# snarkify/sirius

Measured on AMD Instinct MI355X. Metric: IVC fold-steps/s (CycleFold IVC::next hot path, Poseidon-shaped synthetic trace, 2^k rows), higher is better.
Workload: dtype u256 (modular; 9 x 29-bit / 8 x 32-bit limbs)

## Files before the change

### sirius_amd/csrc/capi.hip

```cpp
#include "../../include/sirius_amd.h"

#include <cstdio>
#include <cstring>
#include <deque>
#include <map>
#include <memory>
#include <set>
#include <thread>
#include <condition_variable>
#include <functional>
#include <mutex>
#include <atomic>
#include <chrono>
#include <string>
#include <vector>

#include "curve.cuh"
#include "decider.h"
#include "devrt.h"
#include "msm.h"
#include "ntt.h"
#include "poseidon.h"
#include "prof.h"
#include "rowprog.h"
// ... 1659 lines not shown
    std::vector<std::pair<size_t, size_t>> runs;
    const std::vector<size_t> need = shard_halo_rows(S, reference_compat);
    for (size_t i = 0; i < need.size();) {
        size_t j = i + 1;
        while (j < need.size() && need[j] == need[j - 1] + 1) ++j;
        runs.emplace_back(need[i], need[j - 1] + 1);
        i = j;
    }
    return guarded([&]() -> int {
        const fe_t *src = reinterpret_cast<const fe_t *>(witness_host);
        fe_t *dst = reinterpret_cast<fe_t *>(dev_copy);
        for (auto &r : runs)
            SRS_HIP_CHECK(hipMemcpy2DAsync(dst + r.first, rows * sizeof(fe_t), src + r.first, rows * sizeof(fe_t), (r.second - r.first) * sizeof(fe_t),
                                           cols, hipMemcpyHostToDevice, (hipStream_t)stream));
        return SRS_OK;
    });
}
size_t srs_structure_num_cross_terms(const srs_structure *S) { return S ? rowprog::degree(S->s) : 0; }
size_t srs_structure_num_challenges(const srs_structure *S) { return S ? rowprog::num_challenges(S->s) : 0; }
size_t srs_structure_num_witness_columns(const srs_structure *S) { return S ? rowprog::num_witness_columns(S->s) : 0; }
int srs_jit_selfcheck(size_t *code_bytes, char *log, size_t log_cap) {
    if constexpr (rt::kEmulated) return fail(SRS_ERR_INVALID, "srs_jit_selfcheck: not part of the emulator build");
    std::string text;
    const bool ok = rowprog::jit_selfcheck(code_bytes, text);
    if (log && log_cap) {
        const size_t n = std::min(text.size(), log_cap - 1);
        std::memcpy(log, text.data(), n);
        log[n] = 0;
    }
    return ok ? SRS_OK : fail(SRS_ERR_INVALID, "srs_jit_selfcheck: hiprtc rejected the emitted form: " + text.substr(0, 400));
}

int srs_structure_kernel_kind(const srs_structure *S, int which) {
    if (!S || which < 0 || which > 2) return -1;
    return rowprog::kernel_kind(S->s, which);
}

size_t srs_structure_program_source(srs_structure *S, int which, char *buf, size_t cap, uint64_t *fingerprint, int *spec_id) {
    if (!S) return 0;
    std::string src;
    rowprog::spec_source(S->s, which, fingerprint, spec_id, src);
    if (buf && cap) {
        size_t n = std::min(src.size(), cap - 1);
        std::memcpy(buf, src.data(), n);
        buf[n] = 0;
    }
    return src.size();
}

static int cross_terms_impl(srs_structure *S, srs_ck *ck, const srs_fe *W1, const srs_fe *W2, const srs_fe *challenges,
                            size_t n_challenges, int space, void *stream, srs_fe *const *T_out, srs_affine *commits_out) {
    if (!S || !W1 || !W2 || (n_challenges && !challenges)) return fail(SRS_ERR_INVALID, "srs_cross_terms: bad argument");
    if (ck && !commits_out) return fail(SRS_ERR_INVALID, "srs_commit_cross_terms: commits_out is NULL");
    int rc = ensure_device();
    if (rc) return rc;
    return guarded([&]() -> int {
        hipStream_t st = (hipStream_t)stream;
        rowprog::Structure *s = S->s;
        const size_t d = rowprog::degree(s), rows = rowprog::rows(s), wlen = rowprog::num_witness_columns(s) * rows;
        if (d == 0) return SRS_OK;
        if (ck && rows > ck->key.global_len)
            return fail(SRS_ERR_TOO_LONG_INPUT, "Can't commit too long input: input len: " + std::to_string(rows) +
                                                    ", but limit is " + std::to_string(ck->key.global_len));
        const bool host = space != SRS_SPACE_DEVICE;
        const bool own_T = host || !T_out;
        size_t need = 1024;
        if (host) need += 2 * Arena::pad(wlen * sizeof(fe_t));
// ... 588 lines not shown
                 srs_fe *W_folded) {
    if (!S || !betas || !delta || !W || !alpha_gamma || !poly_F || !poly_K || !betas_stroke || !e || !lagrange ||
        (n_challenges && !challenges))
        return fail(SRS_ERR_INVALID, "srs_pg_prove: bad argument");
    if (n_instances < 2) return fail(SRS_ERR_INVALID, "You can't fold 0 traces");
    if (n_instances & (n_instances - 1)) return fail(SRS_ERR_INVALID, "instances_to_fold must be a power of two");
    if (ro && ro->h->field != SRS_FIELD_FR) return fail(SRS_ERR_INVALID, "srs_pg_prove: the oracle must be over bn256::Fr");
    if (rowprog::shard_world(S->s) > 1)
        return fail(SRS_ERR_INVALID, "srs_pg_prove: structure is row-sharded (srs_structure_set_shard); use the step-wise calls and add the ranks' polynomials");
    int rc = ensure_device();
    if (rc) return rc;
    return guarded([&]() -> int {
        HostTrace ht("srs_pg_prove");
        hipStream_t st = (hipStream_t)stream;
        rowprog::Structure *s = S->s;
        rowprog::PgSizes z;
        if (!rowprog::pg_sizes(s, n_instances - 1, z)) return fail(SRS_ERR_INVALID, "structure has no gates");
        if (n_betas < z.betas_count) return fail(SRS_ERR_INVALID, "srs_pg_prove: not enough betas");
        if (z.log_domain_K > ntt::FR_S)
            return fail(SRS_ERR_K_TOO_LARGE, "srs_pg_prove (compute_K_from_G): k=" + std::to_string(z.log_domain_K) + " should no larger than F::S=28");
        const size_t wlen = rowprog::num_witness_columns(s) * rowprog::rows(s);
        std::vector<const fe_t *> dW(n_instances), ch(n_instances);
        for (size_t j = 0; j < n_instances; ++j) {
            dW[j] = reinterpret_cast<const fe_t *>(W[j]);
            ch[j] = n_challenges ? reinterpret_cast<const fe_t *>(challenges[j]) : nullptr;
        }
        std::string err;
        size_t n_out = 0;
        const bool closed = rowprog::pg_closed_route(reference_compat);
        const uint32_t n_gates = (uint32_t)rowprog::num_gates(s), levels = (uint32_t)z.betas_count, log_rows = rowprog::log_rows(s);
        rowprog::PgRow0 r0;
        int erc = 0;
        if (closed) {
            erc = rowprog::pg_row0_values(s, true, dW.data(), ch.data(), n_challenges, n_instances, st, r0, err);
            if (erc) return fail(erc, "srs_pg_prove (gates at row 0): " + err);
            ht.mark("row0");
            std::vector<fe_t> c0(n_gates);
            for (uint32_t g = 0; g < n_gates; ++g) c0[g] = r0.vals[(size_t)g * r0.P + r0.one_at];
            rowprog::pg_closed_F(c0.data(), n_gates, log_rows, reinterpret_cast<const fe_t *>(betas), *reinterpret_cast<const fe_t *>(delta), levels,
                                 reinterpret_cast<fe_t *>(poly_F), z.points_F);
        } else {
            erc = rowprog::pg_sum(s, 0, dW.data(), ch.data(), n_challenges, 1, reinterpret_cast<const fe_t *>(betas), n_betas,
                                  reinterpret_cast<const fe_t *>(delta), reference_compat, st, reinterpret_cast<fe_t *>(poly_F), &n_out, err);
            if (erc) return fail(erc, "srs_pg_prove (compute_F): " + err);
        }
        ht.mark("compute_F");
        fe_t alpha, gamma;
        std::memcpy(&alpha, &alpha_gamma[0], 32);
        std::memcpy(&gamma, &alpha_gamma[1], 32);
        if (ro) {
            poseidon::absorb(*ro->h, reinterpret_cast<const fe_t *>(poly_F), z.points_F);
            if (!poseidon::squeeze(*ro->h, 255, SRS_FIELD_FR, alpha, err)) return fail(SRS_ERR_INVALID, "srs_pg_prove (alpha): " + err);
        }
        std::vector<fe_t> bs(z.betas_count);
        {
            fe_t d;
            std::memcpy(&d, delta, 32);
            for (size_t i = 0; i < z.betas_count; ++i) {
                fe_t b;
                std::memcpy(&b, &betas[i], 32);
                bs[i] = Fr::add(b, Fr::mul(alpha, d));
                d = Fr::sqr(d);
            }
        }
        const fe_t f_alpha = rowprog::poly_eval(reinterpret_cast<const fe_t *>(poly_F), z.points_F, alpha);
        ht.mark("alpha,betas'");
        std::vector<fe_t> poly_G(z.points_G);
        rowprog::PgGValues gv;
        const bool k_on_device = n_instances == 2 && z.log_domain_K <= 12;
        std::vector<fe_t> g_vals;
        if (closed)
            rowprog::pg_closed_G(s, r0, bs.data(), levels, poly_G.data(), poly_G.size(), &g_vals);
        else
            erc = rowprog::pg_sum(s, 1, dW.data(), ch.data(), n_challenges, n_instances, bs.data(), bs.size(), nullptr, reference_compat, st,
                                  poly_G.data(), &n_out, err, &f_alpha, k_on_device ? &gv : nullptr);
        if (erc) return fail(erc, "srs_pg_prove (compute_G): " + err);
        if (gv.vals_dev && !rowprog::pg_K_device_ok(gv, z.log_domain_K)) return fail(SRS_ERR_DEVICE, "srs_pg_prove: internal (device K on an unsupported shape)");
        ht.mark("compute_G");
        if (closed && k_on_device && r0.g_int && g_vals.size() <= 32)
            erc = rowprog::pg_K_from_G_values(s, g_vals.data(), (uint32_t)g_vals.size(), f_alpha, z.instances_to_fold, z.log_domain_K, st,
                                              reinterpret_cast<fe_t *>(poly_K), err);
        else if (gv.vals_dev)
            erc = rowprog::pg_K_from_G_device(s, gv, f_alpha, z.instances_to_fold, z.log_domain_K, st, reinterpret_cast<fe_t *>(poly_K), err);
        else
            erc = rowprog::pg_K_from_G(poly_G.data(), poly_G.size(), f_alpha, z.instances_to_fold, z.log_domain_K, st,
                                       reinterpret_cast<fe_t *>(poly_K), err);
        if (erc) return fail(erc, "srs_pg_prove (compute_K_from_G): " + err);
        ht.mark("compute_K");
        const size_t n_K = (size_t)1 << z.log_domain_K;
        if (ro) {
            poseidon::absorb(*ro->h, reinterpret_cast<const fe_t *>(poly_K), n_K);
            if (!poseidon::squeeze(*ro->h, 255, SRS_FIELD_FR, gamma, err)) return fail(SRS_ERR_INVALID, "srs_pg_prove (gamma): " + err);
        }
        ht.mark("gamma");
        const std::vector<fe_t> L = rowprog::lagrange_eval(gamma, (uint32_t)z.lagrange_domain);
        const fe_t zg = Fr::sub(Fr::pow_u64(gamma, (uint64_t)1 << z.lagrange_domain), Fr::one());
        const fe_t kg = rowprog::poly_eval(reinterpret_cast<const fe_t *>(poly_K), n_K, gamma);
        const fe_t ev = Fr::add(Fr::mul(f_alpha, L[0]), Fr::mul(zg, kg));
        if (W_folded) {
            erc = rowprog::lincomb(SRS_FIELD_FR, reinterpret_cast<fe_t *>(W_folded), dW.data(), L.data(), n_instances, wlen, st, err);
            if (erc) return fail(erc, "srs_pg_prove (fold_witness): " + err);
        }
        std::memcpy(&alpha_gamma[0], &alpha, 32);
        std::memcpy(&alpha_gamma[1], &gamma, 32);
        std::memcpy(betas_stroke, bs.data(), bs.size() * sizeof(fe_t));
        std::memcpy(e, &ev, 32);
        std::memcpy(lagrange, L.data(), n_instances * sizeof(fe_t));
        ht.mark("e,L,fold");
        return SRS_OK;
    });
}

static int sangria_prove_impl(srs_structure *S, srs_ck *ck, srs_poseidon *ro, const srs_fe *challenges, size_t n_challenges, srs_fe *W1, srs_fe *W2,
                              const srs_fe *W2_host, const srs_fe *u2_tail, size_t n_u2_tail, srs_fe *E, void *stream, srs_fe *r_io,
                              srs_fe *const *T_dev, srs_affine *cross_term_commits, srs_affine *W_commitments, const srs_affine *E_commitment,
                              srs_affine *folded_commitments, uint64_t *jobs, bool incoming) {
    if (!S || !ck || !W1 || !W2 || !E || !r_io || !T_dev || !cross_term_commits || !W_commitments || !E_commitment || !folded_commitments || !jobs ||
        (n_u2_tail && !u2_tail))
        return fail(SRS_ERR_INVALID, "srs_sangria_prove: bad argument");
    const int curve = ck->key.curve, sf = srs_scalar_field_of(curve);
    if (ro && ro->h->field != (curve == SRS_CURVE_BN256 ? SRS_FIELD_FQ : SRS_FIELD_FR))
// ... 146 lines not shown
```

### sirius_amd/csrc/rowprog.h

```cpp
#pragma once
#include <memory>
#include <string>
#include <vector>

#include "devrt.h"
#include "field.cuh"
#include "rowprog_dev.cuh"

namespace srs {
namespace rowprog {

struct Structure;

Structure *create(int field, uint32_t k, size_t num_selectors, size_t num_fixed, size_t num_advice,
                  const uint8_t *const *selectors, const fe_t *const *fixed, int space_device,
                  const uint64_t *gates, size_t gates_words, size_t num_gates, size_t num_lookups, bool has_vector_lookup,
                  const uint64_t *lookup_exprs, size_t lookup_words, int &rc, std::string &err);
void destroy(Structure *S);
void set_shard(Structure *S, uint32_t rank, uint32_t world);
uint32_t shard_world(const Structure *S);
uint32_t shard_rank(const Structure *S);
void rotation_range(const Structure *S, int32_t *lo, int32_t *hi);
uint32_t log_rows(const Structure *S);
size_t degree(const Structure *S);
size_t num_challenges(const Structure *S);
size_t num_advice(const Structure *S);
size_t num_witness_columns(const Structure *S);
size_t num_lookups(const Structure *S);
size_t rows(const Structure *S);
int field(const Structure *S);

int evaluate(Structure *S, int mode, const fe_t *W1_dev, const fe_t *W2_dev, const fe_t *challenges_host, size_t n_ch,
             fe_t *const *out_dev_ptrs_host, hipStream_t st, std::string &err, bool sync = true);

struct PgSizes {
    size_t count_with_padding = 0, betas_count = 0, points_F = 0, points_G = 0, instances_to_fold = 0, lagrange_domain = 0;
    uint32_t log_domain_K = 0;
};
bool pg_sizes(const Structure *S, size_t traces_len, PgSizes &out);
std::vector<fe_t> lagrange_eval(const fe_t &X, uint32_t log_n);
fe_t poly_eval(const fe_t *coeffs, size_t n, const fe_t &x);
struct PgRow0 {
    std::vector<fe_t> vals;
    uint32_t P = 0, one_at = 0;
    bool g_int = false;
};
bool pg_closed_route(int compat);
int pg_row0_values(Structure *S, bool fold, const fe_t *const *W_dev, const fe_t *const *challenges_host, size_t n_ch, size_t J, hipStream_t st,
                   PgRow0 &out, std::string &err);
fe_t pg_closed_sum(const fe_t *c, size_t stride, uint32_t n_gates, uint32_t k, const fe_t *w, uint32_t levels);
void pg_closed_F(const fe_t *c, uint32_t n_gates, uint32_t k, const fe_t *betas, const fe_t &delta, uint32_t levels, fe_t *out, size_t n_out);
void pg_closed_G(const Structure *S, const PgRow0 &r0, const fe_t *betas_stroke, uint32_t levels, fe_t *out, size_t n_out,
                 std::vector<fe_t> *point_values = nullptr);
size_t num_gates(const Structure *S);
struct PgGValues {
    const fe_t *vals_dev = nullptr;
    uint32_t n_dev = 0, degree = 0;
    bool skip_one = false;
};
int pg_sum(Structure *S, int mode, const fe_t *const *W_dev, const fe_t *const *challenges_host, size_t n_ch, size_t J,
           const fe_t *weights_in, size_t n_weights, const fe_t *delta, int compat, hipStream_t st, fe_t *out_host,
           size_t *n_out, std::string &err, const fe_t *g_at_one = nullptr, PgGValues *keep_on_device = nullptr);
bool pg_K_device_ok(const PgGValues &g, uint32_t log_domain_K);
int pg_K_from_G_device(Structure *S, const PgGValues &g, const fe_t &f_alpha, size_t instances_to_fold, uint32_t log_domain_K, hipStream_t st,
                       fe_t *out_host, std::string &err);
int pg_K_from_G_values(Structure *S, const fe_t *vals_host, uint32_t n, const fe_t &f_alpha, size_t instances_to_fold, uint32_t log_domain_K,
                       hipStream_t st, fe_t *out_host, std::string &err);
int pg_K_from_G(const fe_t *polyG_host, size_t nG, const fe_t &f_alpha, size_t instances_to_fold, uint32_t log_domain_K,
                hipStream_t st, fe_t *out_host, std::string &err);
int lincomb(int field, fe_t *out, const fe_t *const *w_dev, const fe_t *coefs, size_t J, size_t n, hipStream_t st, std::string &err,
            uint32_t rank = 0, uint32_t world = 1);
int lincomb_rows(int field, fe_t *out, const fe_t *const *w_dev, const fe_t *coefs, size_t J, const uint32_t *rows_dev, size_t n_rows, size_t cols,
                 size_t col_len, hipStream_t st, std::string &err);

const char *spec_source(Structure *S, int which, uint64_t *fingerprint, int *spec_id, std::string &buf);
int kernel_kind(const Structure *S, int which);
bool jit_selfcheck(size_t *code_bytes, std::string &log);

int lookup_coeff_1(Structure *S, const fe_t *advice_dev, const fe_t &r, fe_t *const *ls, fe_t *const *ts, fe_t *const *ms,
                   hipStream_t st, std::string &err);
void lookup_coeff_2(int field, const fe_t *l, const fe_t *t, const fe_t *m, const fe_t &r, size_t n, fe_t *h, fe_t *g, hipStream_t st);
size_t log_derivative_mismatches(Structure *S, const fe_t *W_dev, hipStream_t st);
void assigned_invert(int field, const fe_t *num, const fe_t *den, const uint8_t *has_den, size_t n, fe_t *out, hipStream_t st);

size_t count_mismatch(const fe_t *a_dev, const fe_t *b_dev , size_t n, hipStream_t st);

void fold_w(int field, fe_t *out, const fe_t *w1, const fe_t *w2, const fe_t &r, size_t n, hipStream_t st);
int fold_e(int field, fe_t *out, const fe_t *e, const fe_t *const *t_dev_ptrs_host, size_t n_terms, const fe_t &r, size_t n,
           hipStream_t st, std::string &err);

}
}
```

### sirius_amd/csrc/rowprog.hip

```cpp
#include "rowprog.h"
#include "rowprog_compile.h"
#include "ntt.h"
#include "prof.h"
#include "jit.h"
#include "tuning.h"

#include <algorithm>
#include <cstring>
#include <map>
#include <mutex>
#include <tuple>

namespace srs {
namespace rowprog {

template <class F>
__device__ __forceinline__ fe_t interp(fe_t *slots, const Insn *__restrict__ prog, uint32_t n_insn, uint32_t result,
                                       const RowCtx &C, uint32_t row, uint32_t pt, const fe_t *__restrict__ U) {
    const uint32_t tid = threadIdx.x, nthr = blockDim.x, mask = C.rows - 1;
    for (uint32_t ip = 0; ip < n_insn; ++ip) {
        const Insn in = prog[ip];
        fe_t r;
        if (in.op <= I_LD_ADV) {
            uint32_t rr = (row + (uint32_t)(int32_t)in.b) & mask;
            if (in.op == I_LD_SEL) r = ld_sel<F>(C, in.a, rr);
            else if (in.op == I_LD_FIX) r = ld_fix<F>(C, in.a, rr);
            else r = ld_adv<F>(C, in.a, rr, pt);
        } else {
            fe_t a = (in.a & UNIFORM_BIT) ? U[in.a & ~UNIFORM_BIT] : slots[in.a * nthr + tid];
            if (in.op <= I_MUL) {
                fe_t b = (in.b & UNIFORM_BIT) ? U[in.b & ~UNIFORM_BIT] : slots[in.b * nthr + tid];
                r = in.op == I_ADD ? F::add(a, b) : (in.op == I_SUB ? F::sub(a, b) : F::mul(a, b));
            } else if (in.op == I_SQR) {
                r = F::sqr(a);
// ... 668 lines not shown
        "    const fe_t l0 = ld_fix<F>(C, 0, (row + 0u) & mask);\n"
        "    fe_t l1, s1; adv_affine<F>(C, 0, (row + 1u) & mask, l1, s1);\n"
        "    for (uint32_t pt = 0; pt < npts; ++pt) {\n"
        "        const fe_t *__restrict__ U = Uall + (size_t)pt * nu;\n"
        "        const f29_t x0 = G::unpack(l0), x1 = G::unpack(l1);\n"
        "        const f29_t x2 = mul29_ni<F>(x0, x1);\n"
        "        const f29_t x3 = sqr29_ni<F>(x2);\n"
        "        const f29_t x4 = G::normalize(G::template sub_lazy<3, 0>(G::normalize(G::add_lazy(x3, x2)), x3));\n"
        "        const f29_t x5 = G::mul(x4, G::unpack(U[0]));\n"
        "        sw_store(acc, pt, accumulate ? G::normalize(G::add_lazy(sw_load(acc, pt), x5)) : x5);\n"
        "        l1 = F::add(l1, s1);\n    }\n}\n";
    for (int field = 0; field < 2; ++field) {
        size_t bytes = 0;
        if (!jit::compile_only(jit_translation_unit(fn, field, true), &bytes, log)) return false;
        if (code_bytes) *code_bytes = bytes;
    }
    return true;
}

struct Structure : Compiled {
    int field = 0;
    uint32_t k = 0;
    size_t rows = 0, num_selectors = 0, num_fixed = 0, num_advice = 0;
    size_t num_lookups = 0;
    bool has_vector_lookup = false;
    int pg_spec_id = -1;
    GateProg *d_gate_progs = nullptr;
    uint8_t **d_sel_ptrs = nullptr;
    fe_t **d_fix_ptrs = nullptr;
    std::vector<void *> owned;
    fe_t *d_vinv = nullptr, *d_vinv29 = nullptr;
    fe_t *d_kM[2] = {nullptr, nullptr};
    Arena arena;
    std::vector<uint8_t> host_stage;
    uint32_t shard_rank = 0, shard_world = 1;
};

static int match_spec(const Program &p) {
    if (!p.sweep_ok) return -1;
    int id = -1;
    for (size_t i = 0; i < sizeof(kSpecs) / sizeof(kSpecs[0]); ++i)
        if (kSpecs[i].fingerprint == p.fingerprint && kSpecs[i].id >= 0) id = kSpecs[i].id;
    return id;
}

static void *resident(Structure &S, const void *src, size_t bytes, hipMemcpyKind kind = hipMemcpyHostToDevice, size_t spare = 0) {
    void *d = nullptr;
    SRS_HIP_CHECK(hipMalloc(&d, bytes + spare));
    S.owned.push_back(d);
    if (bytes) SRS_HIP_CHECK(hipMemcpy(d, src, bytes, kind));
    return d;
}

Structure *create(int field, uint32_t k, size_t num_selectors, size_t num_fixed, size_t num_advice,
                  const uint8_t *const *selectors, const fe_t *const *fixed, int space_device,
                  const uint64_t *gates, size_t gates_words, size_t num_gates, size_t num_lookups, bool has_vector_lookup,
                  const uint64_t *lookup_exprs, size_t lookup_words, int &rc, std::string &err) {
    std::unique_ptr<Structure, void (*)(Structure *)> S(new Structure(), &destroy);
    if (!compile_structure(field, num_selectors, num_fixed, num_advice, gates, gates_words, num_gates, num_lookups, has_vector_lookup,
                           lookup_exprs, lookup_words, *S, rc, err))
        return nullptr;
    S->field = field;
    S->k = k;
    S->rows = (size_t)1 << k;
    S->num_selectors = num_selectors;
    S->num_fixed = num_fixed;
// ... 22 lines not shown
    }
    rc = 5;
    auto upload_program = [&](Program &p) {
        if (!p.insns.empty()) p.d_insns = (Insn *)resident(*S, p.insns.data(), p.insns.size() * sizeof(Insn));
    };
    for (auto &lp : S->lookup_progs) upload_program(lp);
    upload_program(S->cross);
    upload_program(S->plain_compressed);
    upload_program(S->plain_homogeneous);
    for (auto &gp : S->gate_progs) upload_program(gp);
    if (!S->vinv.empty()) {
        S->d_vinv = (fe_t *)resident(*S, S->vinv.data(), S->vinv.size() * sizeof(fe_t));
        const FieldOps f{field};
        std::vector<fe_t> v29(S->vinv);
        for (auto &x : v29)
            for (int k = 0; k < 5; ++k) x = f.add(x, x);
        S->d_vinv29 = (fe_t *)resident(*S, v29.data(), v29.size() * sizeof(fe_t));
    }
    const hipMemcpyKind kind = space_device ? hipMemcpyDeviceToDevice : hipMemcpyHostToDevice;
    std::vector<uint8_t *> selp(num_selectors);
    std::vector<fe_t *> fixp(num_fixed);
    for (size_t i = 0; i < num_selectors; ++i) selp[i] = (uint8_t *)resident(*S, selectors[i], S->rows, kind);
    for (size_t i = 0; i < num_fixed; ++i) fixp[i] = (fe_t *)resident(*S, fixed[i], S->rows * sizeof(fe_t), kind);
    S->d_sel_ptrs = (uint8_t **)resident(*S, selp.data(), num_selectors * sizeof(void *), hipMemcpyHostToDevice, sizeof(void *));
    S->d_fix_ptrs = (fe_t **)resident(*S, fixp.data(), num_fixed * sizeof(void *), hipMemcpyHostToDevice, sizeof(void *));
    rc = 0;
    return S.release();
}

void destroy(Structure *S) {
    if (!S) return;
    jit::release(S->cross.jit);
    for (void *p : S->owned) (void)hipFree(p);
    S->arena.release();
    delete S;
}

void set_shard(Structure *S, uint32_t rank, uint32_t world) {
    S->shard_rank = rank;
    S->shard_world = world ? world : 1;
}
uint32_t shard_world(const Structure *S) { return S->shard_world; }
uint32_t shard_rank(const Structure *S) { return S->shard_rank; }
void rotation_range(const Structure *S, int32_t *lo, int32_t *hi) { *lo = S->min_rot; *hi = S->max_rot; }
uint32_t log_rows(const Structure *S) { return S->k; }
size_t degree(const Structure *S) { return S->degree; }
size_t num_challenges(const Structure *S) { return S->s_num_challenges; }
size_t num_advice(const Structure *S) { return S->num_advice; }
size_t num_witness_columns(const Structure *S) { return S->num_advice + 5 * S->num_lookups; }
size_t num_lookups(const Structure *S) { return S->num_lookups; }
size_t rows(const Structure *S) { return S->rows; }
size_t num_gates(const Structure *S) { return S->gate_progs.size(); }
int field(const Structure *S) { return S->field; }

template <class F>
static void launch_rowprog(const DevArgs &A, uint32_t nslots, hipStream_t st) {
    uint32_t blocks = (A.ctx.local_rows + RP_THREADS - 1) / RP_THREADS;
    if (nslots <= 8) SRS_LAUNCH((k_rowprog<F, 8>), (blocks), (RP_THREADS), 0, st, A);
    else if (nslots <= 10) SRS_LAUNCH((k_rowprog<F, 10>), (blocks), (RP_THREADS), 0, st, A);
    else if (nslots <= 12) SRS_LAUNCH((k_rowprog<F, 12>), (blocks), (RP_THREADS), 0, st, A);
    else if (nslots <= 16) SRS_LAUNCH((k_rowprog<F, 16>), (blocks), (RP_THREADS), 0, st, A);
    else if (nslots <= 24) SRS_LAUNCH((k_rowprog<F, 24>), (blocks), (RP_THREADS), 0, st, A);
    else SRS_LAUNCH((k_rowprog<F, 32>), (blocks), (RP_THREADS), 0, st, A);
}

int kernel_kind(const Structure *S, int which) {
    if (which == 2) return S->pg_spec_id >= 0 ? 1 : 0;
    const Program &p = which == 0 ? S->cross : S->plain_compressed;
    if (p.spec_id >= 0) return 1;
    if (p.jit.function) return 2;
    return 0;
}

const char *spec_source(Structure *S, int which, uint64_t *fingerprint, int *spec_id, std::string &buf) {
    if (which >= 3 && (size_t)(which - 3) >= S->gate_progs.size()) { buf.clear(); return buf.c_str(); }
    Program &p = which >= 3 ? S->gate_progs[which - 3] : (which == 0 ? S->cross : (which == 1 ? S->plain_compressed : S->plain_homogeneous));
    buf = emit_spec_source(p, "spec_fn", false);
    buf += emit_sweep_source(p, "spec_fn_sweep", false);
    if (fingerprint) *fingerprint = p.fingerprint;
    if (spec_id) *spec_id = p.spec_id;
    if (spec_id && p.spec_id < 0 && p.jit.function) *spec_id = -2;
    return buf.c_str();
}

static int evaluate_prog(Structure *S, Program &p, int mode, const fe_t *W1_dev, const fe_t *W2_dev, const fe_t *challenges_host,
                         size_t n_ch, fe_t *const *out_dev_ptrs_host, hipStream_t st, std::string &err, bool sync = true);
int evaluate(Structure *S, int mode, const fe_t *W1_dev, const fe_t *W2_dev, const fe_t *challenges_host, size_t n_ch,
             fe_t *const *out_dev_ptrs_host, hipStream_t st, std::string &err, bool sync) {
    Program &p = mode == 0 ? S->cross : (mode == 1 ? S->plain_compressed : S->plain_homogeneous);
    return evaluate_prog(S, p, mode, W1_dev, W2_dev, challenges_host, n_ch, out_dev_ptrs_host, st, err, sync);
}
static int evaluate_prog(Structure *S, Program &p, int mode, const fe_t *W1_dev, const fe_t *W2_dev, const fe_t *challenges_host,
                         size_t n_ch, fe_t *const *out_dev_ptrs_host, hipStream_t st, std::string &err, bool sync) {
    FieldOps f{S->field};
    const uint32_t d = mode == 0 ? (uint32_t)S->degree : 0;
    const uint32_t npts = mode == 0 ? d + 1 : 1;
    const uint32_t nout = mode == 0 ? d : 1;
    if (mode == 0 && d == 0) return 0;
    if (p.nslots > 32) { err = "row program needs more than 32 live registers"; return 4; }
// ... 182 lines not shown
    uint32_t deg = levels > k ? levels - k : 0;
    for (uint32_t b = 0; b < k && b < levels; ++b) mul_linear(sum, deg, Fr::add(Fr::one(), betas[b]), deltas[b]);
    for (size_t m = 0; m < n_out; ++m) out[m] = m <= deg ? sum[m] : Fr::zero();
}

void pg_closed_G(const Structure *S, const PgRow0 &r0, const fe_t *betas_stroke, uint32_t levels, fe_t *out, size_t n_out, std::vector<fe_t> *point_values) {
    const uint32_t n_gates = (uint32_t)S->gate_progs.size(), P = r0.P;
    std::vector<fe_t> val(P);
    for (uint32_t p = 0; p < P; ++p) val[p] = pg_closed_sum(r0.vals.data() + p, P, n_gates, S->k, betas_stroke, levels);
    if (point_values) *point_values = val;
    for (size_t m = 0; m < n_out; ++m) out[m] = Fr::zero();
    if (r0.g_int) {
        const uint32_t dG = P - 1;
        FieldOps f{0};
        const std::vector<fe_t> vinv = !S->vinv_g.empty() ? S->vinv_g : (dG ? inverse_vandermonde_rows(f, dG) : std::vector<fe_t>());
        out[0] = val[0];
        for (uint32_t k = 1; k <= dG && k < n_out; ++k) {
            fe_t acc = Fr::zero();
            for (uint32_t j = 0; j < P; ++j) acc = Fr::add(acc, Fr::mul(vinv[(size_t)(k - 1) * P + j], val[j]));
            out[k] = acc;
        }
        return;
    }
    const fe_t winv = ntt::omega(ilog2(P), true), inv_P = Fr::inv(Fr::from_u64(P));
    fe_t wk = Fr::one();
    for (uint32_t k = 0; k < P && k < n_out; ++k) {
        fe_t acc = Fr::zero(), x = Fr::one();
        for (uint32_t p = 0; p < P; ++p) { acc = Fr::add(acc, Fr::mul(val[p], x)); x = Fr::mul(x, wk); }
        out[k] = Fr::mul(acc, inv_P);
        wk = Fr::mul(wk, winv);
    }
}

int pg_row0_values(Structure *S, bool fold, const fe_t *const *W_dev, const fe_t *const *challenges_host, size_t n_ch, size_t J, hipStream_t st,
                   PgRow0 &out, std::string &err) {
    if (S->field != 0) { err = "ProtoGalaxy polynomials need the 2-adic field bn256::Fr"; return 4; }
    if (J == 0 || J > JMAX) { err = "unsupported number of traces"; return 4; }
    PgSizes sz;
    if (!pg_sizes(S, fold ? J - 1 : 1, sz)) { err = "structure has no gates"; return 4; }
    FieldOps f{0};
    const bool g_int = fold && J == 2 && tuning::get_or(tuning::PG_G_FFT, 0) == 0;
    const uint32_t P = !fold ? 1u : (g_int ? (uint32_t)S->max_gate_degree + 1 : (uint32_t)sz.points_G);
    const uint32_t n_gates = (uint32_t)S->gate_progs.size();
    out.P = P;
    out.g_int = g_int;
    out.one_at = g_int ? 1u : 0u;
    std::vector<fe_t> wcoef;
    std::vector<std::vector<fe_t>> ch_pt(P, std::vector<fe_t>(n_ch ? n_ch : 1, Fr::zero()));
    if (fold) {
        wcoef.resize((size_t)P * J);
        const fe_t w = g_int ? Fr::one() : ntt::omega(ilog2(P), false);
        fe_t x = g_int ? Fr::zero() : Fr::one();
        for (uint32_t p = 0; p < P; ++p) {
            if (!g_int || n_ch) {
                std::vector<fe_t> L = lagrange_eval(x, (uint32_t)sz.lagrange_domain);
                for (size_t j = 0; j < J; ++j) {
                    wcoef[(size_t)p * J + j] = L[j];
                    for (size_t c = 0; c < n_ch; ++c)
                        ch_pt[p][c] = Fr::add(ch_pt[p][c], Fr::mul(challenges_host[j][c], L[j]));
                }
            }
            x = g_int ? Fr::add(x, Fr::one()) : Fr::mul(x, w);
        }
    } else {
        for (size_t c = 0; c < n_ch; ++c) ch_pt[0][c] = challenges_host[0][c];
    }
    const bool sweep = S->pg_spec_id >= 0 && S->k >= 10 && (!fold || g_int) && P <= DMAX + 1;
    const uint32_t lpt = 8;
    uint32_t max_slots = 1;
    std::vector<GateProg> gp(n_gates);
    std::vector<fe_t> utab;
    for (uint32_t g = 0; g < n_gates; ++g) {
        Program &p = S->gate_progs[g];
        max_slots = std::max(max_slots, p.nslots);
        const size_t nu = p.uops.size() ? p.uops.size() : 1;
        gp[g].prog = p.d_insns;
        gp[g].n_insn = (uint32_t)p.insns.size();
        gp[g].result = p.result;
        gp[g].n_uniform = (uint32_t)nu;
        gp[g].utab_off = (uint32_t)utab.size();
        utab.resize(utab.size() + nu * P * (sweep ? lpt + 1 : 1u));
        fe_t *tab = utab.data() + gp[g].utab_off;
        for (uint32_t lp = 0; lp < P; ++lp)
            if (!eval_uniform(p, f, ch_pt[lp].data(), n_ch, 0, false, 0, tab + (size_t)lp * nu, err)) return 7;
        if (sweep) std::memcpy(tab + (size_t)lpt * P * nu, tab, (size_t)P * nu * sizeof(fe_t));
    }
    if (max_slots > 32) { err = "row program needs more than 32 live registers"; return 4; }
    Arena &A = S->arena;
    A.reserve(Arena::pad((wcoef.size() + 1) * sizeof(fe_t)) + Arena::pad((utab.size() + 1) * sizeof(fe_t)) + Arena::pad(gp.size() * sizeof(GateProg)) +
              Arena::pad(((size_t)n_gates * P + 1) * sizeof(fe_t)) + 4096);
    A.reset();
    fe_t *d_coef = A.take<fe_t>(wcoef.size() + 1);
    fe_t *d_utab = A.take<fe_t>(utab.size() + 1);
    GateProg *d_gp = A.take<GateProg>(gp.size());
    fe_t *d_vals = A.take<fe_t>((size_t)n_gates * P + 1);
    if (fold && !g_int) SRS_HIP_CHECK(hipMemcpyAsync(d_coef, wcoef.data(), wcoef.size() * sizeof(fe_t), hipMemcpyHostToDevice, st));
    SRS_HIP_CHECK(hipMemcpyAsync(d_utab, utab.data(), utab.size() * sizeof(fe_t), hipMemcpyHostToDevice, st));
    SRS_HIP_CHECK(hipMemcpyAsync(d_gp, gp.data(), gp.size() * sizeof(GateProg), hipMemcpyHostToDevice, st));
    PgArgs a;
// ... 532 lines not shown
    bool zero_z = false;
    const fe_t *tab = k_domain_table_dev(log_domain_K, instances_to_fold, zero_z);
    if (zero_z) { err = "Z(X) must be not equal to 0"; return 4; }
    fe_t *&M = S->d_kM[g.skip_one ? 1 : 0];
    if (!M) {
        FieldOps f{0};
        std::vector<fe_t> full((size_t)n_nodes * n_nodes);
        if (g.skip_one) {
            full = !S->vinv_g1.empty() ? S->vinv_g1 : inverse_vandermonde_at(f, g.degree, 1);
        } else {
            const std::vector<fe_t> rows = !S->vinv_g.empty() ? S->vinv_g : (g.degree ? inverse_vandermonde_rows(f, g.degree) : std::vector<fe_t>());
            for (uint32_t j = 0; j < n_nodes; ++j) full[j] = j == 0 ? Fr::one() : Fr::zero();
            for (size_t i = 0; i < rows.size(); ++i) full[n_nodes + i] = rows[i];
        }
        SRS_HIP_CHECK(hipMalloc((void **)&M, full.size() * sizeof(fe_t)));
        S->owned.push_back(M);
        SRS_HIP_CHECK(hipMemcpy(M, full.data(), full.size() * sizeof(fe_t), hipMemcpyHostToDevice));
    }
    static thread_local ThreadArena scratch;
    scratch.reserve(Arena::pad((size_t)count * sizeof(fe_t)) + 256);
    scratch.reset();
    fe_t *d_out = scratch.take<fe_t>(count);
    const uint32_t threads = std::max<uint32_t>(64u, std::min<uint32_t>(256u, count));
    SRS_LAUNCH(k_pg_K_small, ((count + threads - 1) / threads), (threads), 0, st, g.vals_dev, g.n_dev, f_alpha, g.skip_one ? 1 : 0, (const fe_t *)M,
               n_nodes, f_alpha, tab, count, d_out);
    ntt::run(d_out, log_domain_K, count, 1, true, true, st);
    SRS_HIP_CHECK(hipMemcpyAsync(out_host, d_out, (size_t)count * sizeof(fe_t), hipMemcpyDeviceToHost, st));
    SRS_HIP_CHECK(hipStreamSynchronize(st));
    SRS_HIP_CHECK(hipGetLastError());
    prof::collect();
    return 0;
}

int pg_K_from_G_values(Structure *S, const fe_t *vals_host, uint32_t n, const fe_t &f_alpha, size_t instances_to_fold, uint32_t log_domain_K,
                       hipStream_t st, fe_t *out_host, std::string &err) {
    static thread_local ThreadArena scratch;
    scratch.reserve(Arena::pad((size_t)n * sizeof(fe_t)) + 256);
    scratch.reset();
    fe_t *d_vals = scratch.take<fe_t>(n);
    SRS_HIP_CHECK(hipMemcpyAsync(d_vals, vals_host, (size_t)n * sizeof(fe_t), hipMemcpyHostToDevice, st));
    PgGValues g;
    g.vals_dev = d_vals;
    g.n_dev = n;
    g.degree = n - 1;
    g.skip_one = false;
    return pg_K_from_G_device(S, g, f_alpha, instances_to_fold, log_domain_K, st, out_host, err);
}

size_t count_mismatch(const fe_t *a_dev, const fe_t *b_dev, size_t n, hipStream_t st) {
    if (!n) return 0;
    uint32_t *d = nullptr, h = 0;
    SRS_HIP_CHECK(hipMalloc((void **)&d, sizeof(uint32_t)));
    SRS_HIP_CHECK(hipMemsetAsync(d, 0, sizeof(uint32_t), st));
    SRS_LAUNCH(k_count_mismatch, ((uint32_t)((n + 255) / 256)), (256), 0, st, a_dev, b_dev, n, d);
    SRS_HIP_CHECK(hipMemcpyAsync(&h, d, sizeof(uint32_t), hipMemcpyDeviceToHost, st));
    SRS_HIP_CHECK(hipStreamSynchronize(st));
    (void)hipFree(d);
    return h;
}

int lookup_coeff_1(Structure *S, const fe_t *advice_dev, const fe_t &r, fe_t *const *ls, fe_t *const *ts, fe_t *const *ms,
                   hipStream_t st, std::string &err) {
    const size_t L = S->num_lookups;
    if (!L) { err = "structure has no lookup arguments"; return 4; }
    const uint32_t n = (uint32_t)S->rows;
    for (size_t i = 0; i < 2 * L; ++i) {
// ... 117 lines not shown
```

### sirius_amd/csrc/tuning.h

```cpp
#pragma once
#include <cstdint>

namespace srs {
namespace tuning {

enum Id : int {
    MSM_SORT = 0,
    MSM_L0,
    MSM_WIDE,
    MSM_WIDE_MIN,
    MSM_SLOTS,
    MSM_SLOT_LOG,
    MSM_EXPECT_OVF,
    MSM_QUAD_MAX,
    COMMIT_CHUNKS,
    PG_F_EVAL,
    PG_G_FFT,
    JIT_ALWAYS,
    NO_JIT,
    MSM_COMPACT,
    PG_COMPAT_TREE,
    N_TUNABLES
};

constexpr int64_t UNSET = INT64_MIN;

int64_t get(Id id);
inline int64_t get_or(Id id, int64_t dflt) {
    const int64_t v = get(id);
    return v == UNSET ? dflt : v;
}
int set(const char *name, int64_t value);
int64_t get_by_name(const char *name, int *found);
void reset();
const char *name_of(int id);

}
}
```

### sirius_amd/csrc/tuning.hip

```cpp
#include "tuning.h"

#include <atomic>
#include <cstring>

namespace srs {
namespace tuning {

static std::atomic<int64_t> g_val[N_TUNABLES];
static const char *const kNames[N_TUNABLES] = {"msm_sort", "msm_l0", "msm_wide", "msm_wide_min", "msm_slots", "msm_slot_log", "msm_expect_ovf",
                                               "msm_quad_max", "commit_chunks", "pg_f_eval", "pg_g_fft", "jit_always", "no_jit", "msm_compact", "pg_compat_tree"};
static struct Init {
    Init() { for (auto &v : g_val) v.store(UNSET, std::memory_order_relaxed); }
} g_init;

int64_t get(Id id) { return g_val[id].load(std::memory_order_relaxed); }
const char *name_of(int id) { return id >= 0 && id < N_TUNABLES ? kNames[id] : nullptr; }
static int find(const char *name) {
    if (!name) return -1;
    for (int i = 0; i < N_TUNABLES; ++i)
        if (std::strcmp(kNames[i], name) == 0) return i;
    return -1;
}
int set(const char *name, int64_t value) {
    const int i = find(name);
    if (i < 0) return -1;
    g_val[i].store(value, std::memory_order_relaxed);
    return 0;
}
int64_t get_by_name(const char *name, int *found) {
    const int i = find(name);
    if (found) *found = i >= 0;
    return i < 0 ? UNSET : get((Id)i);
}
void reset() { for (auto &v : g_val) v.store(UNSET, std::memory_order_relaxed); }

}
}
```

Measured before the change: 99.87.

## Evaluate ProtoGalaxy row-0 gates and small K polynomial on host in closed form

For small gate counts, row-0 gate values are now computed on the host. A tiny gather kernel pulls only the referenced cells into pinned memory, and an interpreter evaluates the gate programs there instead of launching the device row-0 kernels. For small K domains, K is obtained by host synthetic division of G minus F(alpha)·L0 by the vanishing polynomial, with cached inverse constants, replacing the device kernel, NTT and copies. The goal is to cut kernel launch and sync latency in the fold step. The cost is host serial field arithmetic, plus new tunables to turn each route off.

```diff
diff --git a/sirius_amd/csrc/capi.hip b/sirius_amd/csrc/capi.hip
--- a/sirius_amd/csrc/capi.hip
+++ b/sirius_amd/csrc/capi.hip
@@ -1715,7 +1715,7 @@
 }
 
 int srs_structure_kernel_kind(const srs_structure *S, int which) {
-    if (!S || which < 0 || which > 2) return -1;
+    if (!S || which < 0 || which > 4) return -1;
     return rowprog::kernel_kind(S->s, which);
 }
 
@@ -2370,9 +2370,9 @@
         rowprog::PgRow0 r0;
         int erc = 0;
         if (closed) {
-            erc = rowprog::pg_row0_values(s, true, dW.data(), ch.data(), n_challenges, n_instances, st, r0, err);
+            erc = rowprog::pg_row0_values(s, true, dW.data(), ch.data(), n_challenges, n_instances, st, r0, err, true);
             if (erc) return fail(erc, "srs_pg_prove (gates at row 0): " + err);
-            ht.mark("row0");
+            ht.mark(rowprog::kernel_kind(s, 3) == 1 ? "row0 (host)" : "row0 (device)");
             std::vector<fe_t> c0(n_gates);
             for (uint32_t g = 0; g < n_gates; ++g) c0[g] = r0.vals[(size_t)g * r0.P + r0.one_at];
             rowprog::pg_closed_F(c0.data(), n_gates, log_rows, reinterpret_cast<const fe_t *>(betas), *reinterpret_cast<const fe_t *>(delta), levels,
@@ -2415,7 +2415,13 @@
         if (erc) return fail(erc, "srs_pg_prove (compute_G): " + err);
         if (gv.vals_dev && !rowprog::pg_K_device_ok(gv, z.log_domain_K)) return fail(SRS_ERR_DEVICE, "srs_pg_prove: internal (device K on an unsupported shape)");
         ht.mark("compute_G");
-        if (closed && k_on_device && r0.g_int && g_vals.size() <= 32)
+        const size_t n_G = r0.g_int ? g_vals.size() : 0;
+        const bool k_closed = closed && k_on_device && r0.g_int && rowprog::pg_K_closed_ok(n_G, z.instances_to_fold, z.log_domain_K);
+        rowprog::pg_note_K_route(s, k_closed ? 1 : 0);
+        if (k_closed)
+            erc = rowprog::pg_K_from_G_closed(s, poly_G.data(), std::min(n_G, poly_G.size()), f_alpha, z.instances_to_fold, z.log_domain_K,
+                                              reinterpret_cast<fe_t *>(poly_K), err);
+        else if (closed && k_on_device && r0.g_int && g_vals.size() <= 32)
             erc = rowprog::pg_K_from_G_values(s, g_vals.data(), (uint32_t)g_vals.size(), f_alpha, z.instances_to_fold, z.log_domain_K, st,
                                               reinterpret_cast<fe_t *>(poly_K), err);
         else if (gv.vals_dev)
@@ -2424,7 +2430,7 @@
             erc = rowprog::pg_K_from_G(poly_G.data(), poly_G.size(), f_alpha, z.instances_to_fold, z.log_domain_K, st,
                                        reinterpret_cast<fe_t *>(poly_K), err);
         if (erc) return fail(erc, "srs_pg_prove (compute_K_from_G): " + err);
-        ht.mark("compute_K");
+        ht.mark(k_closed ? "compute_K (host)" : "compute_K (device)");
         const size_t n_K = (size_t)1 << z.log_domain_K;
         if (ro) {
             poseidon::absorb(*ro->h, reinterpret_cast<const fe_t *>(poly_K), n_K);
diff --git a/sirius_amd/csrc/pg_host.h b/sirius_amd/csrc/pg_host.h
--- /dev/null
+++ b/sirius_amd/csrc/pg_host.h
@@ -0,0 +1,112 @@
+#pragma once
+#include <string>
+#include <vector>
+
+#include "rowprog_dev.cuh"
+
+namespace srs {
+namespace rowprog {
+
+struct Row0Cell {
+    uint32_t kind, col, row, pad;
+};
+
+struct Row0Plan {
+    std::vector<Row0Cell> cells;
+    std::vector<std::vector<int32_t>> cell_of;
+};
+
+inline void row0_plan_add(Row0Plan &plan, const Insn *prog, size_t n_insn, uint32_t rows) {
+    std::vector<int32_t> of(n_insn, -1);
+    for (size_t ip = 0; ip < n_insn; ++ip) {
+        const Insn &in = prog[ip];
+        if (in.op > I_LD_ADV) continue;
+        const uint32_t rr = (0u + (uint32_t)(int32_t)in.b) & (rows - 1);
+        int32_t at = -1;
+        for (size_t c = 0; c < plan.cells.size() && at < 0; ++c)
+            if (plan.cells[c].kind == in.op && plan.cells[c].col == in.a && plan.cells[c].row == rr) at = (int32_t)c;
+        if (at < 0) {
+            at = (int32_t)plan.cells.size();
+            plan.cells.push_back(Row0Cell{in.op, in.a, rr, 0u});
+        }
+        of[ip] = at;
+    }
+    plan.cell_of.push_back(std::move(of));
+}
+
+inline void row0_fold_cells(const Row0Plan &plan, const fe_t *gathered, uint32_t J, bool half, const fe_t *coef, uint32_t pt, fe_t *out) {
+    const size_t n = plan.cells.size();
+    for (size_t c = 0; c < n; ++c) {
+        if (plan.cells[c].kind != I_LD_ADV) { out[c] = gathered[c]; continue; }
+        const fe_t w0 = gathered[c];
+        if (coef) {
+            fe_t r = Fr::mul(coef[0], w0);
+            for (uint32_t j = 1; j < J; ++j) r = Fr::add(r, Fr::mul(coef[j], gathered[(size_t)j * n + c]));
+            out[c] = r;
+        } else if (J == 2 && half) {
+            const fe_t w1 = gathered[n + c];
+            const fe_t a = Fr::halve(Fr::add(w0, w1)), b = Fr::halve(Fr::sub(w0, w1));
+            out[c] = pt ? Fr::add(a, Fr::mul(b, Fr::from_u64(pt))) : a;
+        } else {
+            out[c] = w0;
+        }
+    }
+}
+
+inline fe_t row0_interp(const Insn *prog, size_t n_insn, uint32_t result, const int32_t *cell_of, const fe_t *cells, const fe_t *U, fe_t *slots) {
+    for (size_t ip = 0; ip < n_insn; ++ip) {
+        const Insn &in = prog[ip];
+        fe_t r;
+        if (in.op <= I_LD_ADV) {
+            r = cells[cell_of[ip]];
+        } else {
+            const fe_t a = (in.a & UNIFORM_BIT) ? U[in.a & ~UNIFORM_BIT] : slots[in.a];
+            if (in.op <= I_MUL) {
+                const fe_t b = (in.b & UNIFORM_BIT) ? U[in.b & ~UNIFORM_BIT] : slots[in.b];
+                r = in.op == I_ADD ? Fr::add(a, b) : (in.op == I_SUB ? Fr::sub(a, b) : Fr::mul(a, b));
+            } else if (in.op == I_SQR) {
+                r = Fr::sqr(a);
+            } else if (in.op == I_DBL) {
+                r = Fr::dbl(a);
+            } else {
+                r = Fr::neg(a);
+            }
+        }
+        slots[in.dst] = r;
+    }
+    return (result & UNIFORM_BIT) ? U[result & ~UNIFORM_BIT] : slots[result];
+}
+
+inline bool pg_K_host_ok(size_t n_G, size_t n, uint32_t log_domain_K) {
+    if (n == 0 || (n & (n - 1)) || log_domain_K > 12) return false;
+    const size_t N = (size_t)1 << log_domain_K;
+    return n <= N && n_G < N + n + 1;
+}
+inline int pg_K_host(const fe_t *G, size_t n_G, const fe_t &f_alpha, size_t n, uint32_t log_domain_K, const fe_t &inv_n, const fe_t &inv_c1,
+                     fe_t *out, std::string &err) {
+    if (!pg_K_host_ok(n_G, n, log_domain_K)) { err = "K in closed form: deg K >= 2^log_domain_K or a domain the instances do not divide"; return 4; }
+    const size_t N = (size_t)1 << log_domain_K;
+    std::vector<fe_t> d(G, G + n_G);
+    if (d.size() < n) d.resize(n, Fr::zero());
+    const fe_t l0 = Fr::mul(f_alpha, inv_n);
+    for (size_t i = 0; i < n; ++i) d[i] = Fr::sub(d[i], l0);
+    for (size_t i = 0; i < N; ++i) out[i] = Fr::zero();
+    for (size_t i = d.size(); i-- > n;) {
+        out[i - n] = d[i];
+        d[i - n] = Fr::add(d[i - n], d[i]);
+    }
+    fe_t r_at_1 = Fr::zero();
+    for (size_t i = 0; i < n; ++i) r_at_1 = Fr::add(r_at_1, d[i]);
+    if (!Fr::is_zero(r_at_1)) { err = "internal: K in closed form: G(1) != F(alpha), the remainder of G - F(alpha) L_0 by Z does not vanish at 1"; return 5; }
+    bool exact = true;
+    for (size_t i = 0; i < n; ++i) exact = exact && Fr::is_zero(d[i]);
+    if (exact) return 0;
+    for (size_t i = 0; i < n; ++i) {
+        const fe_t t = Fr::mul(d[i], inv_c1);
+        for (size_t j = i; j < N; j += n) out[j] = Fr::add(out[j], t);
+    }
+    return 0;
+}
+
+}
+}
diff --git a/sirius_amd/csrc/rowprog.h b/sirius_amd/csrc/rowprog.h
--- a/sirius_amd/csrc/rowprog.h
+++ b/sirius_amd/csrc/rowprog.h
@@ -47,7 +47,7 @@
 };
 bool pg_closed_route(int compat);
 int pg_row0_values(Structure *S, bool fold, const fe_t *const *W_dev, const fe_t *const *challenges_host, size_t n_ch, size_t J, hipStream_t st,
-                   PgRow0 &out, std::string &err);
+                   PgRow0 &out, std::string &err, bool allow_host = false);
 fe_t pg_closed_sum(const fe_t *c, size_t stride, uint32_t n_gates, uint32_t k, const fe_t *w, uint32_t levels);
 void pg_closed_F(const fe_t *c, uint32_t n_gates, uint32_t k, const fe_t *betas, const fe_t &delta, uint32_t levels, fe_t *out, size_t n_out);
 void pg_closed_G(const Structure *S, const PgRow0 &r0, const fe_t *betas_stroke, uint32_t levels, fe_t *out, size_t n_out,
@@ -66,6 +66,10 @@
                        fe_t *out_host, std::string &err);
 int pg_K_from_G_values(Structure *S, const fe_t *vals_host, uint32_t n, const fe_t &f_alpha, size_t instances_to_fold, uint32_t log_domain_K,
                        hipStream_t st, fe_t *out_host, std::string &err);
+bool pg_K_closed_ok(size_t n_G, size_t instances_to_fold, uint32_t log_domain_K);
+void pg_note_K_route(Structure *S, int route);
+int pg_K_from_G_closed(Structure *S, const fe_t *polyG_host, size_t n_G, const fe_t &f_alpha, size_t instances_to_fold, uint32_t log_domain_K,
+                       fe_t *out_host, std::string &err);
 int pg_K_from_G(const fe_t *polyG_host, size_t nG, const fe_t &f_alpha, size_t instances_to_fold, uint32_t log_domain_K,
                 hipStream_t st, fe_t *out_host, std::string &err);
 int lincomb(int field, fe_t *out, const fe_t *const *w_dev, const fe_t *coefs, size_t J, size_t n, hipStream_t st, std::string &err,
diff --git a/sirius_amd/csrc/rowprog.hip b/sirius_amd/csrc/rowprog.hip
--- a/sirius_amd/csrc/rowprog.hip
+++ b/sirius_amd/csrc/rowprog.hip
@@ -1,5 +1,6 @@
 #include "rowprog.h"
 #include "rowprog_compile.h"
+#include "pg_host.h"
 #include "ntt.h"
 #include "prof.h"
 #include "jit.h"
@@ -734,6 +735,12 @@
     fe_t *d_vinv = nullptr, *d_vinv29 = nullptr;
     fe_t *d_kM[2] = {nullptr, nullptr};
     Arena arena;
+    Row0Plan row0_plan;
+    bool row0_plan_built = false;
+    Row0Cell *d_row0_cells = nullptr;
+    fe_t *h_row0 = nullptr;
+    size_t h_row0_cap = 0;
+    int last_row0_route = -1, last_K_route = -1;
     std::vector<uint8_t> host_stage;
     uint32_t shard_rank = 0, shard_world = 1;
 };
@@ -822,6 +829,7 @@
     if (!S) return;
     jit::release(S->cross.jit);
     for (void *p : S->owned) (void)hipFree(p);
+    if (S->h_row0) (void)hipHostFree(S->h_row0);
     S->arena.release();
     delete S;
 }
@@ -855,6 +863,8 @@
 }
 
 int kernel_kind(const Structure *S, int which) {
+    if (which == 3) return S->last_row0_route;
+    if (which == 4) return S->last_K_route;
     if (which == 2) return S->pg_spec_id >= 0 ? 1 : 0;
     const Program &p = which == 0 ? S->cross : S->plain_compressed;
     if (p.spec_id >= 0) return 1;
@@ -1103,8 +1113,109 @@
     }
 }
 
+struct Row0GatherArgs {
+    const Row0Cell *cells;
+    uint32_t n_cells, J, rows;
+    const uint8_t *const *sel;
+    const fe_t *const *fix;
+    const fe_t *W[JMAX];
+    fe_t *out;
+};
+__global__ void SRS_KERNEL_BOUNDS(64, 1) k_pg_row0_gather(Row0GatherArgs A) {
+    const uint32_t t = blockIdx.x * blockDim.x + threadIdx.x;
+    if (t >= A.n_cells * A.J) return;
+    const uint32_t c = t % A.n_cells, j = t / A.n_cells;
+    const Row0Cell q = A.cells[c];
+    fe_t v = Fr::zero();
+    if (q.kind == I_LD_ADV) {
+        const fe_t *w = A.W[0];
+        for (uint32_t i = 1; i < JMAX; ++i)
+            if (i == j) w = A.W[i];
+        v = w[(size_t)q.col * A.rows + q.row];
+    } else if (j == 0) {
+        v = q.kind == I_LD_SEL ? (A.sel[q.col][q.row] ? Fr::one() : Fr::zero()) : A.fix[q.col][q.row];
+    }
+    A.out[t] = v;
+}
+
+static int pg_row0_values_host(Structure *S, bool fold, bool g_int, uint32_t P, const fe_t *const *W_dev, const std::vector<std::vector<fe_t>> &ch_pt,
+                               size_t n_ch, const std::vector<fe_t> &wcoef, size_t J, hipStream_t st, PgRow0 &out, std::string &err) {
+    FieldOps f{0};
+    const uint32_t n_gates = (uint32_t)S->gate_progs.size(), Jf = (uint32_t)(fold ? J : 1);
+    if (!S->row0_plan_built) {
+        Row0Plan plan;
+        for (const Program &p : S->gate_progs) row0_plan_add(plan, p.insns.data(), p.insns.size(), (uint32_t)S->rows);
+        S->d_row0_cells = (Row0Cell *)resident(*S, plan.cells.data(), plan.cells.size() * sizeof(Row0Cell), hipMemcpyHostToDevice, sizeof(Row0Cell));
+        S->row0_plan = std::move(plan);
+        S->row0_plan_built = true;
+    }
+    const Row0Plan &plan = S->row0_plan;
+    const uint32_t n_cells = (uint32_t)plan.cells.size();
+    const size_t n_vals = (size_t)n_cells * Jf;
+    if (n_vals) {
+        if (S->h_row0_cap < n_vals) {
+            if (S->h_row0) (void)hipHostFree(S->h_row0);
+            S->h_row0 = nullptr;
+            S->h_row0_cap = 0;
+            SRS_HIP_CHECK(hipHostMalloc((void **)&S->h_row0, n_vals * sizeof(fe_t), hipHostMallocDefault));
+            S->h_row0_cap = n_vals;
+        }
+        Arena &A = S->arena;
+        A.reserve(Arena::pad(n_vals * sizeof(fe_t)) + 256);
+        A.reset();
+        Row0GatherArgs a;
+        a.cells = S->d_row0_cells;
+        a.n_cells = n_cells;
+        a.J = Jf;
+        a.rows = (uint32_t)S->rows;
+        a.sel = S->d_sel_ptrs;
+        a.fix = S->d_fix_ptrs;
+        for (uint32_t j = 0; j < JMAX; ++j) a.W[j] = j < Jf ? W_dev[j] : nullptr;
+        a.out = A.take<fe_t>(n_vals);
+        {
+            prof::Scope ps("pg_row0_gather", st, n_vals);
+            SRS_LAUNCH(k_pg_row0_gather, ((uint32_t)((n_vals + 63) / 64)), (64), 0, st, a);
+        }
+        SRS_HIP_CHECK(hipMemcpyAsync(S->h_row0, a.out, n_vals * sizeof(fe_t), hipMemcpyDeviceToHost, st));
+    }
+    std::vector<size_t> uoff(n_gates + 1, 0);
+    uint32_t max_slots = 1;
+    for (uint32_t g = 0; g < n_gates; ++g) {
+        const Program &p = S->gate_progs[g];
+        uoff[g + 1] = uoff[g] + (p.uops.size() ? p.uops.size() : 1) * P;
+        max_slots = std::max(max_slots, p.nslots);
+    }
+    std::vector<fe_t> utab(uoff[n_gates]);
+    for (uint32_t g = 0; g < n_gates; ++g) {
+        const Program &p = S->gate_progs[g];
+        const size_t nu = p.uops.size() ? p.uops.size() : 1;
+        for (uint32_t lp = 0; lp < P; ++lp)
+            if (!eval_uniform(p, f, ch_pt[lp].data(), n_ch, 0, false, 0, utab.data() + uoff[g] + (size_t)lp * nu, err)) {
+                if (n_vals) (void)hipStreamSynchronize(st);
+                return 7;
+            }
+    }
+    if (n_vals) {
+        SRS_HIP_CHECK(hipStreamSynchronize(st));
+        SRS_HIP_CHECK(hipGetLastError());
+        prof::collect();
+    }
+    std::vector<fe_t> cells(n_cells ? n_cells : 1), slots(max_slots);
+    out.vals.resize((size_t)n_gates * P);
+    for (uint32_t lp = 0; lp < P; ++lp) {
+        row0_fold_cells(plan, S->h_row0, Jf, g_int, (fold && !g_int) ? wcoef.data() + (size_t)lp * J : nullptr, lp, cells.data());
+        for (uint32_t g = 0; g < n_gates; ++g) {
+            const Program &p = S->gate_progs[g];
+            const size_t nu = p.uops.size() ? p.uops.size() : 1;
+            out.vals[(size_t)g * P + lp] = row0_interp(p.insns.data(), p.insns.size(), p.result, plan.cell_of[g].data(), cells.data(),
+                                                       utab.data() + uoff[g] + (size_t)lp * nu, slots.data());
+        }
+    }
+    return 0;
+}
+
 int pg_row0_values(Structure *S, bool fold, const fe_t *const *W_dev, const fe_t *const *challenges_host, size_t n_ch, size_t J, hipStream_t st,
-                   PgRow0 &out, std::string &err) {
+                   PgRow0 &out, std::string &err, bool allow_host) {
     if (S->field != 0) { err = "ProtoGalaxy polynomials need the 2-adic field bn256::Fr"; return 4; }
     if (J == 0 || J > JMAX) { err = "unsupported number of traces"; return 4; }
     PgSizes sz;
@@ -1136,6 +1247,11 @@
     } else {
         for (size_t c = 0; c < n_ch; ++c) ch_pt[0][c] = challenges_host[0][c];
     }
+    if (allow_host && S->shard_world <= 1 && (int64_t)S->gate_progs.size() * P <= tuning::get_or(tuning::PG_ROW0_HOST_MAX, tuning::PG_ROW0_HOST_MAX_DEFAULT)) {
+        S->last_row0_route = 1;
+        return pg_row0_values_host(S, fold, g_int, P, W_dev, ch_pt, n_ch, wcoef, J, st, out, err);
+    }
+    if (allow_host) S->last_row0_route = 0;
     const bool sweep = S->pg_spec_id >= 0 && S->k >= 10 && (!fold || g_int) && P <= DMAX + 1;
     const uint32_t lpt = 8;
     uint32_t max_slots = 1;
@@ -1734,6 +1850,34 @@
     return 0;
 }
 
+void pg_note_K_route(Structure *S, int route) { S->last_K_route = route; }
+bool pg_K_closed_ok(size_t n_G, size_t instances_to_fold, uint32_t log_domain_K) {
+    return log_domain_K <= 8 && pg_K_host_ok(n_G, instances_to_fold, log_domain_K) && tuning::get_or(tuning::PG_K_HOST, 1) != 0;
+}
+int pg_K_from_G_closed(Structure *S, const fe_t *polyG_host, size_t n_G, const fe_t &f_alpha, size_t instances_to_fold, uint32_t log_domain_K,
+                       fe_t *out_host, std::string &err) {
+    if (!pg_K_host_ok(n_G, instances_to_fold, log_domain_K)) { err = "internal: K in closed form outside its guard"; return 5; }
+    struct Consts { fe_t inv_n, inv_c1; bool zero_z = false; };
+    static std::mutex mu;
+    static std::map<std::pair<uint32_t, size_t>, Consts> cache;
+    Consts c;
+    {
+        std::lock_guard<std::mutex> lk(mu);
+        auto it = cache.find({log_domain_K, instances_to_fold});
+        if (it == cache.end()) {
+            Consts n;
+            const fe_t c1 = Fr::sub(Fr::pow_u64(ntt::zeta(), (uint64_t)1 << log_domain_K), Fr::one());
+            n.zero_z = Fr::is_zero(c1);
+            n.inv_n = Fr::inv(Fr::from_u64(instances_to_fold));
+            n.inv_c1 = n.zero_z ? Fr::zero() : Fr::inv(c1);
+            it = cache.emplace(std::make_pair(log_domain_K, instances_to_fold), n).first;
+        }
+        c = it->second;
+    }
+    if (c.zero_z) { err = "Z(X) must be not equal to 0"; return 4; }
+    return pg_K_host(polyG_host, n_G, f_alpha, instances_to_fold, log_domain_K, c.inv_n, c.inv_c1, out_host, err);
+}
+
 int pg_K_from_G_values(Structure *S, const fe_t *vals_host, uint32_t n, const fe_t &f_alpha, size_t instances_to_fold, uint32_t log_domain_K,
                        hipStream_t st, fe_t *out_host, std::string &err) {
     static thread_local ThreadArena scratch;
diff --git a/sirius_amd/csrc/tuning.h b/sirius_amd/csrc/tuning.h
--- a/sirius_amd/csrc/tuning.h
+++ b/sirius_amd/csrc/tuning.h
@@ -20,8 +20,11 @@
     NO_JIT,
     MSM_COMPACT,
     PG_COMPAT_TREE,
+    PG_ROW0_HOST_MAX,
+    PG_K_HOST,
     N_TUNABLES
 };
+constexpr int64_t PG_ROW0_HOST_MAX_DEFAULT = 32;
 
 constexpr int64_t UNSET = INT64_MIN;
 
diff --git a/sirius_amd/csrc/tuning.hip b/sirius_amd/csrc/tuning.hip
--- a/sirius_amd/csrc/tuning.hip
+++ b/sirius_amd/csrc/tuning.hip
@@ -8,7 +8,8 @@
 
 static std::atomic<int64_t> g_val[N_TUNABLES];
 static const char *const kNames[N_TUNABLES] = {"msm_sort", "msm_l0", "msm_wide", "msm_wide_min", "msm_slots", "msm_slot_log", "msm_expect_ovf",
-                                               "msm_quad_max", "commit_chunks", "pg_f_eval", "pg_g_fft", "jit_always", "no_jit", "msm_compact", "pg_compat_tree"};
+                                               "msm_quad_max", "commit_chunks", "pg_f_eval", "pg_g_fft", "jit_always", "no_jit", "msm_compact", "pg_compat_tree",
+                                               "pg_row0_host_max", "pg_k_host"};
 static struct Init {
     Init() { for (auto &v : g_val) v.store(UNSET, std::memory_order_relaxed); }
 } g_init;
```

New measurement: 101.1, median of 6. 1.01x the previous value.
